# mehrnazmo/VIforSSMs

Measured on AMD Instinct MI355X. Metric: latent-state transitions/sec (batch_dims×T per step), AR(1) T=5000, 1/2/4/8 GPU, higher is better.
Workload: dtype bf16

## Files before the change

viforssms_amd/csrc/flow_v5.hip:

```cpp
#include "flow5_api.hpp"

#ifndef VISSM_FLOW5_NS
#define VISSM_FLOW5_NS flow5
#define VISSM_FLOW5_BASE_UNIT 1
#endif

#include <cstdlib>
#ifndef VISSM_ABL_STORES
#define VISSM_ABL_STORES 0
#endif

namespace vissm {
namespace VISSM_FLOW5_NS {

constexpr int P = 16;
constexpr int HP = 64;
constexpr int S = 16;
constexpr int NW = 4;
constexpr int NT = 64 * NW;
constexpr int UW = 128;
constexpr int DTH = 56;

typedef __bf16 bf4 __attribute__((ext_vector_type(4)));
typedef __bf16 bf8 __attribute__((ext_vector_type(8)));
// ... 1057 lines not shown
  }
}

constexpr int NW2 = 8;
constexpr int NT2 = 64 * NW2;
__device__ __forceinline__ float swap_hi_lo(float v) {
  const auto r = __builtin_amdgcn_permlane32_swap(__builtin_bit_cast(unsigned, v), __builtin_bit_cast(unsigned, v),
                                                  false, false);
  return __builtin_bit_cast(float, static_cast<unsigned>(r[1]));
}
constexpr int KP2 = 8;
#ifndef VISSM_NODU_FENCES
#define VISSM_NODU_FENCES 1
#endif
template <bool FZ>
__device__ __forceinline__ void fence2() {
  if constexpr (FZ) fence();
}
#ifndef VISSM_BWD2_AHEAD
#define VISSM_BWD2_AHEAD 2
#endif
#ifndef VISSM_BWD2_AHEAD_VAR
#define VISSM_BWD2_AHEAD_VAR 6
#endif
#ifndef VISSM_BWD2_TAIL_DU
#define VISSM_BWD2_TAIL_DU 5
#endif
#ifndef VISSM_BWD2_TAIL_FZ
#define VISSM_BWD2_TAIL_FZ 59
#endif
#ifndef VISSM_BWD2_TAIL_NODU
#define VISSM_BWD2_TAIL_NODU 4
#endif
constexpr int kSgMfma = 0x008, kSgDsRead = 0x100;
template <int ID, int N, int M>
__device__ __forceinline__ void sg_batch() {
  __builtin_amdgcn_sched_group_barrier(kSgDsRead, N, ID);
#pragma unroll
  for (int i = 0; i < N; ++i) __builtin_amdgcn_sched_group_barrier(kSgMfma, M, ID);
}
template <int ID, int NR, int NM>
__device__ __forceinline__ void sg_seq() {
  __builtin_amdgcn_sched_group_barrier(kSgDsRead, NR, ID);
  __builtin_amdgcn_sched_group_barrier(kSgMfma, NM, ID);
}

__device__ __forceinline__ bf8 cat8(bf4 a, bf4 b) {
  return __builtin_shufflevector(a, b, 0, 1, 2, 3, 4, 5, 6, 7);
}
__device__ __forceinline__ bf8 tr_frag2(const __bf16* img, int hb, int g, int c) {
  return cat8(tr_read(img, hb, g, c), tr_read(img + P * HP, hb, g, c));
}

template <bool FZ, bool DU, bool TF, int NPR = 1, bool SB = false>
__global__ __launch_bounds__(NT2, 2) void bwd2_kernel(KArgs a, const float* __restrict__ u, const float* __restrict__ C,
                                                      const float* __restrict__ tht, const float* __restrict__ gout,
                                                      const float* __restrict__ dls, const bf8* __restrict__ img,
                                                      const float* __restrict__ cst, float* __restrict__ du,
                                                      float* __restrict__ dC_slab, float* __restrict__ dth_slab,
                                                      float* __restrict__ dW_slab, float* __restrict__ halo,
                                                      const u4* __restrict__ thf, FzArgs fz = FzArgs{}) {
  static_assert(!SB || NPR == 2, "the split backward chain goes with the split recompute");
  constexpr int NH = 1, KB = 1, JB = 1, NP = 1;
  constexpr bool LOF = NPR == 2 && !kLoFoldOff;
  constexpr bool AH =
      VISSM_BWD2_AHEAD && NPR == 1 && (FZ || TF) && (VISSM_BWD2_AHEAD_VAR & (FZ ? 4 : DU ? 2 : 1)) != 0;
  constexpr int TAIL = (VISSM_BWD2_AHEAD >= 2 && NPR == 1 && TF)
                           ? (FZ ? VISSM_BWD2_TAIL_FZ : DU ? VISSM_BWD2_TAIL_DU : VISSM_BWD2_TAIL_NODU) : 0;
  constexpr int PO = FZ ? P - 1 : P;
  constexpr int QW2 = P + KP2;
  constexpr int UWN = NPR == 2 ? 48 : 64;
  __shared__ Shared<NH, KB, JB, NP> sh;
  __shared__ __bf16 timg[NW2][2][2 * P * HP];
  __shared__ float dthl[NW2][S][DTH];
  __shared__ __attribute__((aligned(16))) float dths[NW2][4];
  __shared__ float carry[NW2][S][KP2];
  __shared__ float uwin[NW2][2][UWN];
  __shared__ float gwin[NW2][2][P];
  __shared__ float gsc[NPR == 2 ? 1 : NW2][2][P];
  __shared__ float dscr[NW2][2][KP2][QW2];
  constexpr bool ZLS = FZ && NPR == 1;
  __shared__ float zls[ZLS ? NW2 : 1][ZLS ? S : 1][P];
  constexpr int RO = NPR == 2 ? 10 : 0, NLO = RO + (SB ? 10 : 0);
  __shared__ bf8 slo[NLO > 0 ? NLO : 1][64];
  __shared__ bf8 swe[NPR == 2 ? 4 : 1][16];
  __shared__ float zcar[FZ ? NW2 : 1][FZ ? S : 1];
  if constexpr (NPR == 2) {
    constexpr int NFR = Shared<NH, KB, JB, NP>::NFR;
    for (int i = threadIdx.x; i < NFR * 64; i += NT2) sh.img[i >> 6][0][i & 63] = img[((i >> 6) * 2) * 64 + (i & 63)];
    for (int i = threadIdx.x; i < NLO * 64; i += NT2) {
      const int j = i >> 6;
      const int f = j < 8 ? j
                  : j < 10 ? 16 * NH + 4 * KB + 2 * JB + (j - 8)
                  : j < 18 ? 8 * NH + (j - 10)
                           : 16 * NH + 4 * KB + (j - 18);
      slo[j][i & 63] = img[(f * 2 + 1) * 64 + (i & 63)];
    }
    for (int i = threadIdx.x; i < 4 * 16; i += NT2) swe[i >> 4][i & 15] = img[((16 * NH + (i >> 4)) * 2 + 1) * 64 + (i & 15)];
    for (int i = threadIdx.x; i < Shared<NH, KB, JB, NP>::NCST; i += NT2) sh.cst[i] = cst[i];
  } else {
    load_shared<NH, KB, JB, NP, NT2>(sh, img, cst);
  }
  if constexpr (FZ) {
    if constexpr (ZLS)
      for (int i = threadIdx.x; i < NW2 * S * P; i += NT2) (&zls[0][0][0])[i] = 0.f;
    for (int i = threadIdx.x; i < NW2 * S; i += NT2) (&zcar[0][0])[i] = 0.f;
  }
  for (int i = threadIdx.x; i < NW2 * S * DTH; i += NT2) (&dthl[0][0][0])[i] = 0.f;
  for (int i = threadIdx.x; i < NW2 * S * KP2; i += NT2) (&carry[0][0][0])[i] = 0.f;
  for (int i = threadIdx.x; i < NW2 * 2 * KP2 * QW2; i += NT2) (&dscr[0][0][0][0])[i] = 0.f;
  __syncthreads();
// ... 3 lines not shown
  const int chn = __builtin_amdgcn_readfirstlane(item % a.n_chunks);
  if (grp >= a.n_groups) return;
  const int m_lo = chn * a.CH, m_hi = min(a.Lh, m_lo + a.CH);
  const int b_lo = grp * a.S, nb = min(a.S, a.B - b_lo);
  __bf16* const im0 = timg[w][0];
  __bf16* const im1 = timg[w][1];
  const unsigned* whp = reinterpret_cast<const unsigned*>(&sh.cst[NH * HP]);

  f4 dW[4][4], dWe[4], dWh[4];
#pragma unroll
  for (int i = 0; i < 4; ++i) {
#pragma unroll
    for (int o = 0; o < 4; ++o) dW[i][o] = f4{0.f, 0.f, 0.f, 0.f};
    dWe[i] = f4{0.f, 0.f, 0.f, 0.f};
    dWh[i] = f4{0.f, 0.f, 0.f, 0.f};
  }
  const int fwc = 16 * NH + 4 * KB;
  bf8 sel_p;
#pragma unroll
  for (int jj = 0; jj < 8; ++jj) sel_p[jj] = (__bf16)((4 * g + (jj & 3) == c) ? 1.f : 0.f);

  const float ldl = (!FZ && lane < nb) ? dls[b_lo + lane] : 0.f;
  float lt0 = 0.f, lt1 = 0.f, lis = 0.f;
  if constexpr (FZ) {
    if (lane < nb) {
      const float* tp = fz.theta + static_cast<size_t>(b_lo + lane) * 3;
      lt0 = tp[0];
      lt1 = tp[1];
      lis = __expf(-tp[2]);
    }
  }
  const int m_start = (FZ && chn > 0) ? m_lo - PO : m_lo;
  const int nu = a.k + P;
  for (int m0 = m_start; m0 < m_hi; m0 += PO) {
    const bool discard = FZ && m0 < m_lo;
    const int nP = discard ? 0 : min(PO, m_hi - m0), t0 = m0;
    const int nZ = FZ ? min(P, a.Lh - m0) : nP;
    f4 dCa[4];
#pragma unroll
    for (int rb = 0; rb < 4; ++rb) dCa[rb] = f4{0.f, 0.f, 0.f, 0.f};
    float fz_yt = 0.f, fz_bt = 0.f;
    if constexpr (FZ) {
      const int wo = min(max(m0 + c - 1, 0), fz.M - 1);
      fz_yt = fz.obs[wo];
      fz_bt = fz.bin[wo];
    }
    for (int bl = 0; bl < nb; bl += 2) {
      fence2<FZ || (!DU && VISSM_NODU_FENCES)>();
      const bool two = bl + 1 < nb;
      const int blv[2] = {bl, two ? bl + 1 : bl};
      const int bv[2] = {b_lo + blv[0], b_lo + blv[1]};
      f4 X[2][4];
      bf8 tfr[2];
      float fz_yp = fz_yt, fz_bp = fz_bt, fz_zc[2] = {0.f, 0.f};
      {
        float uv[2], gv[2] = {0.f, 0.f};
#pragma unroll
        for (int cb = 0; cb < 2; ++cb) {
          const float* ub = u + static_cast<size_t>(bv[cb]) * a.pL;
          uv[cb] = lane < nu ? ub[clampi(t0 + lane, a.L)] : 0.f;
          if constexpr (!FZ) {
            if (lane < P) gv[cb] = gout[static_cast<size_t>(bv[cb]) * a.pLo + clampi(t0 + lane, a.Lout)];
          }
        }
        if (!two) gv[1] = 0.f;
        const f4* crow = reinterpret_cast<const f4*>(C + static_cast<size_t>(m0 + clampi(c, nZ)) * HP) + g;
        f4 cr[4], tr[2][4];
        if constexpr (TF) {
#pragma unroll
          for (int cb = 0; cb < 2; ++cb) tfr[cb] = __builtin_bit_cast(bf8, thf[2 * static_cast<size_t>(bv[cb]) + (g & 1)]);
        }
#pragma unroll
        for (int rb = 0; rb < 4; ++rb) {
          cr[rb] = crow[4 * rb];
          if constexpr (!TF) {
#pragma unroll
            for (int cb = 0; cb < 2; ++cb)
              tr[cb][rb] = (reinterpret_cast<const f4*>(tht + static_cast<size_t>(bv[cb]) * HP) + g)[4 * rb];
          }
        }
        __builtin_amdgcn_sched_barrier(0);
#pragma unroll
        for (int cb = 0; cb < 2; ++cb) {
          if (UWN == 64 || lane < UWN) uwin[w][cb][lane] = uv[cb];
          if (lane < P) gwin[w][cb][lane] = gv[cb];
#pragma unroll
          for (int rb = 0; rb < 4; ++rb) X[cb][rb] = TF ? cr[rb] : cr[rb] + tr[cb][rb];
        }
        if constexpr (FZ) {
          fz_zc[0] = zcar[w][blv[0]];
          fz_zc[1] = zcar[w][blv[1]];
        }
      }
      u2 i0p[2][4];
      u2 d0p[2][4], d1p[2][4];
      float mu[2], rr[2];
      float uk_e = 0.f;
      {
        f4 acc[2][4];
        fence2<FZ || (!DU && VISSM_NODU_FENCES)>();
        const int gu = (LOF && g == 1) ? 0 : g;
        Fr8<NP> uf[2] = {u_frag<NP>(uwin[w][0], 1, 0, gu, c), u_frag<NP>(uwin[w][1], 1, 0, gu, c)};
        if constexpr (TF) {
          if (g >= 2) {
            uf[0].h = tfr[0];
            uf[1].h = tfr[1];
          }
        }
        if constexpr (AH) {
          bf8 we[4];
#pragma unroll
          for (int ob = 0; ob < 4; ++ob) we[ob] = sh.img[16 * NH + ob][0][lane];
          if constexpr ((TAIL & 8) != 0) __builtin_amdgcn_sched_barrier(0);
#pragma unroll
          for (int ob = 0; ob < 4; ++ob)
#pragma unroll
            for (int cb = 0; cb < 2; ++cb) acc[cb][ob] = mfma32(we[ob], uf[cb].h, X[cb][ob]);
          if constexpr ((TAIL & 8) == 0) sg_batch<1, 4, 2>();
        } else {
#pragma unroll
          for (int ob = 0; ob < 4; ++ob) {
            const Fr8<NP> wf = wfrag(sh, 16 * NH + ob, lane);
            bf8 wel = {};
            if constexpr (NPR == 2 && !LOF) {
              const bf8 v = swe[ob][c];
              if (g == 0) wel = v;
            }
#pragma unroll
            for (int cb = 0; cb < 2; ++cb) {
              acc[cb][ob] = X[cb][ob];
              if constexpr (NPR == 2 && !LOF) acc[cb][ob] = mfma32(wel, uf[cb].h, acc[cb][ob]);
              acc[cb][ob] = mm<NP>(wf, uf[cb], acc[cb][ob]);
            }
          }
        }
#pragma unroll
        for (int cb = 0; cb < 2; ++cb)
#pragma unroll
          for (int rb = 0; rb < 4; ++rb) {
            float e[4] = {0.f, 0.f, 0.f, 0.f};
#pragma unroll
            for (int r = 0; r < 4; ++r) {
              if (VISSM_DERIV16 >= 1) X[cb][rb][r] = 4 * rb + r < NR ? elu_dv(acc[cb][rb][r], e[r]) : 0.f;
              else X[cb][rb][r] = 4 * rb + r < NR ? elu_fast<true>(acc[cb][rb][r]) : 0.f;
            }
            if (VISSM_DERIV16 >= 1) {
              d0p[cb][rb] = u2{pk_f16(e[0], e[1]), 4 * rb + 2 < NR ? pk_f16(e[2], e[3]) : 0u};
              pin_pair(d0p[cb][rb]);
            }
          }
        fence2<FZ || (!DU && VISSM_NODU_FENCES)>();
#pragma unroll
        for (int cb = 0; cb < 2; ++cb) {
          if (g == 3) X[cb][3][3] = 1.f;
#pragma unroll
          for (int ob = 0; ob < 4; ++ob) acc[cb][ob] = f4{0.f, 0.f, 0.f, 0.f};
        }
#pragma unroll
        for (int ks = 0; ks < 2; ++ks) {
          Fr8<NP> xf[2] = {chain_frag<NP>(X[0], ks), chain_frag<NP>(X[1], ks)};
          if constexpr (AH) {
            bf8 wq[4];
#pragma unroll
            for (int ob = 0; ob < 4; ++ob) wq[ob] = sh.img[ob * 2 + ks][0][lane];
#pragma unroll
            for (int ob = 0; ob < 4; ++ob)
#pragma unroll
              for (int cb = 0; cb < 2; ++cb) acc[cb][ob] = mfma32(wq[ob], xf[cb].h, acc[cb][ob]);
            if (ks == 0) sg_batch<2, 4, 2>();
            else sg_batch<3, 4, 2>();
          } else {
#pragma unroll
            for (int ob = 0; ob < 4; ++ob) {
              const Fr8<NP> wf = wfrag(sh, ob * 2 + ks, lane);
#pragma unroll
              for (int cb = 0; cb < 2; ++cb) {
                if constexpr (NPR == 2) acc[cb][ob] = mfma32(slo[ob * 2 + ks][lane], xf[cb].h, acc[cb][ob]);
                acc[cb][ob] = mm<NP>(wf, xf[cb], acc[cb][ob]);
              }
            }
          }
        }
#pragma unroll
        for (int cb = 0; cb < 2; ++cb) {
          put_image<NP>(im0 + cb * P * HP, nullptr, X[cb], g, c);
          if (VISSM_DERIV16 == 0) {
#pragma unroll
            for (int rb = 0; rb < 4; ++rb) i0p[cb][rb] = u2{cvt2(X[cb][rb][0], X[cb][rb][1]), cvt2(X[cb][rb][2], X[cb][rb][3])};
          }
        }
#pragma unroll
        for (int cb = 0; cb < 2; ++cb)
#pragma unroll
          for (int rb = 0; rb < 4; ++rb) {
            float e[4] = {0.f, 0.f, 0.f, 0.f};
#pragma unroll
            for (int r = 0; r < 4; ++r) {
              if (VISSM_DERIV16 >= 2) X[cb][rb][r] = 4 * rb + r < NR ? elu_dv(acc[cb][rb][r], e[r]) : 0.f;
              else X[cb][rb][r] = 4 * rb + r < NR ? elu_fast<true>(acc[cb][rb][r]) : 0.f;
            }
            if (VISSM_DERIV16 >= 2) {
              d1p[cb][rb] = u2{pk_f16(e[0], e[1]), 4 * rb + 2 < NR ? pk_f16(e[2], e[3]) : 0u};
              pin_pair(d1p[cb][rb]);
            }
          }
        fence2<FZ || (!DU && VISSM_NODU_FENCES)>();
        const int fh = 16 * NH + 4 * KB + 2 * JB;
        f4 d[2] = {f4{0.f, 0.f, 0.f, 0.f}, f4{0.f, 0.f, 0.f, 0.f}};
#pragma unroll
        for (int cb = 0; cb < 2; ++cb)
          if (g == 3) X[cb][3][3] = 1.f;
        if constexpr (FZ && (TAIL & 32) != 0) uk_e = uwin[w][g >> 1][c + a.k];
        if constexpr (AH) {
          const bf8 wh[2] = {sh.img[fh][0][lane], sh.img[fh + 1][0][lane]};
#pragma unroll
          for (int ks = 0; ks < 2; ++ks)
#pragma unroll
            for (int cb = 0; cb < 2; ++cb) d[cb] = mfma32(wh[ks], chain_frag<NP>(X[cb], ks).h, d[cb]);
          sg_batch<4, 2, 2>();
        } else {
#pragma unroll
          for (int ks = 0; ks < 2; ++ks) {
            const Fr8<NP> wf = wfrag(sh, fh + ks, lane);
#pragma unroll
            for (int cb = 0; cb < 2; ++cb) {
              const Fr8<NP> xk = chain_frag<NP>(X[cb], ks);
              if constexpr (NPR == 2 && !LOF) d[cb] = mfma32(slo[8 + ks][lane], xk.h, d[cb]);
              d[cb] = mm<NP>(wf, xk, d[cb]);
            }
          }
        }
#pragma unroll
        for (int cb = 0; cb < 2; ++cb) {
          mu[cb] = LOF ? d[cb][0] + d[cb][2] : d[cb][0];
          rr[cb] = LOF ? d[cb][1] + d[cb][3] : d[cb][1];
          put_image<NP>(im1 + cb * P * HP, nullptr, X[cb], g, c);
        }
      }
      const bool pv = c < nP;
      float gmu[2], gr[2];
      float lsv[2] = {0.f, 0.f};
      if constexpr (FZ) {
        const int hs = g >> 1;
        const bool hv = hs == 0 || two;
        const float mu_h = hs ? mu[1] : mu[0], rr_h = hs ? rr[1] : rr[0];
        const float sig_h = softplus_fast(rr_h) + 1e-10f;
        const float uk = (TAIL & 32) ? uk_e : uwin[w][hs][c + a.k];
        const float x = uk * sig_h + mu_h;
        float xp = row_prev(x);
        const float xn = row_next(x);
        if (c == 0) xp = hs ? fz_zc[1] : fz_zc[0];
        const int bl2 = hs ? blv[1] : blv[0];
        const float th0 = hs ? lane_f(lt0, blv[1]) : lane_f(lt0, blv[0]);
        const float th1 = hs ? lane_f(lt1, blv[1]) : lane_f(lt1, blv[0]);
        const float is = hs ? lane_f(lis, blv[1]) : lane_f(lis, blv[0]);
        const int t = m0 + c;
        const float fh = (pv && t < fz.M) ? 1.f : 0.f;
        const float ft = (pv && t >= 1) ? 1.f : 0.f;
        const float bp = fz_bp * ft;
        const float zt = fh * (xn - th1 * x - th0) * is;
        const float zp = ft * (x - th1 * xp - th0) * is;
        const float de = th1 * zt * is - zp * is - bp * (x - fz_yp) * (fz.iosd * fz.iosd);
        const float gmu_h = hv ? -fz.scale * de : 0.f;
        const float lsg = (t0 + c >= a.Lout - a.n_logsig) ? __builtin_amdgcn_logf(sig_h) * kLn2 : 0.f;
        if ((g & 1) == 0) {
          if constexpr (NPR == 1) gwin[w][hs][c] = gmu_h;
          if (pv && hv) {
            if constexpr (!(VISSM_ABL_STORES & 1)) fz.x[static_cast<size_t>(b_lo + bl2) * (fz.M + 1) + t] = x;
            if constexpr (ZLS) zls[w][bl2][c] += lsg;
          }
        }
        if ((lane & 31) == PO - 1 && (nP == PO || discard) && hv) zcar[w][bl2] = x;
        float dsig = gmu_h * uk;
        if (pv && hv && t0 + c >= a.Lout - a.n_logsig) dsig += -fz.scale * rcp_f(sig_h);
        const float gr_h = dsig * sigmoid_fast(rr_h);
        if ((g & 1) == 0) {
          if constexpr (NPR == 2) {
            if constexpr (DU) gwin[w][hs][c] = gmu_h * sig_h;
          } else {
            gsc[w][hs][c] = sig_h;
          }
        }
        gmu[0] = gmu_h;
        gr[0] = gr_h;
        gmu[1] = swap_hi_lo(gmu_h);
        gr[1] = swap_hi_lo(gr_h);
        if constexpr (!ZLS) {
          const float lsv_h = (pv && hv) ? lsg : 0.f;
          lsv[0] = lsv_h;
          lsv[1] = swap_hi_lo(lsv_h);
        }
#pragma unroll
        for (int cb = 0; cb < 2; ++cb) {
          if (g == 1) {
            const int off = timg_off(c, 4 * 3 + 1);
            *reinterpret_cast<u2*>(im1 + cb * P * HP + off) = u2{cvt2(X[cb][3][0], gmu[cb]), cvt2(gr[cb], X[cb][3][3])};
          }
        }
      } else {
        float sig[2];
#pragma unroll
        for (int cb = 0; cb < 2; ++cb) {
          sig[cb] = softplus_fast(rr[cb]) + 1e-10f;
          gmu[cb] = pv ? gwin[w][cb][c] : 0.f;
        }
#pragma unroll
        for (int cb = 0; cb < 2; ++cb) {
          const float dl = lane_f(ldl, blv[cb]);
          float dsig = gmu[cb] * uwin[w][cb][c + a.k];
          if (pv && (cb == 0 || two) && t0 + c >= a.Lout - a.n_logsig) dsig += dl * rcp_f(sig[cb]);
          gr[cb] = dsig * sigmoid_fast(rr[cb]);
          if (g == 0) {
            if constexpr (NPR == 2) {
              if constexpr (DU) gwin[w][cb][c] = gmu[cb] * sig[cb];
            } else {
              gsc[w][cb][c] = sig[cb];
            }
          }
          if (g == 1) {
            const int off = timg_off(c, 4 * 3 + 1);
            *reinterpret_cast<u2*>(im1 + cb * P * HP + off) = u2{cvt2(X[cb][3][0], gmu[cb]), cvt2(gr[cb], X[cb][3][3])};
          }
        }
      }
      fence2<FZ || (!DU && VISSM_NODU_FENCES)>();
      bf8 i1f[4];
#pragma unroll
      for (int hb = 0; hb < 4; ++hb) i1f[hb] = tr_frag2(im1, hb, g, c);
      if constexpr (!AH) {
#pragma unroll
        for (int hb = 0; hb < 4; ++hb) dWh[hb] = mfma32(i1f[hb], i1f[3], dWh[hb]);
      }
      f4 D[2][4];
      {
        unsigned wvh[4], wvl[4];
#pragma unroll
        for (int rb = 0; rb < 4; ++rb) {
          wvh[rb] = whp[16 * rb + c];
          if constexpr (SB) wvl[rb] = whp[HP + 16 * rb + c];
        }
        const bool g0 = g == 0;
#pragma unroll
        for (int cb = 0; cb < 2; ++cb) {
          const bf4 gf2 = __builtin_bit_cast(bf4, u2{cvt2(g0 ? gmu[cb] : 0.f, g0 ? gr[cb] : 0.f), 0u});
#pragma unroll
          for (int rb = 0; rb < 4; ++rb) {
            const bf4 wa = __builtin_bit_cast(bf4, u2{g0 ? wvh[rb] : 0u, 0u});
            f4 d0 = f4{0.f, 0.f, 0.f, 0.f};
            if constexpr (SB) d0 = mfma16(__builtin_bit_cast(bf4, u2{g0 ? wvl[rb] : 0u, 0u}), gf2, d0);
            D[cb][rb] = mfma16(wa, gf2, d0);
          }
        }
        fence2<FZ || (!DU && VISSM_NODU_FENCES)>();
#pragma unroll
        for (int cb = 0; cb < 2; ++cb) {
#pragma unroll
          for (int rb = 0; rb < 4; ++rb)
#pragma unroll
// ... 37 lines not shown
#pragma unroll
            for (int cb = 0; cb < 2; ++cb) {
              if constexpr (SB) dX[cb][ib] = mfma32(slo[RO + ib * 2 + ks][lane], df[cb].h, dX[cb][ib]);
              dX[cb][ib] = mm<NP>(wb, df[cb], dX[cb][ib]);
            }
          }
        }
      }
      fence2<FZ || (!DU && VISSM_NODU_FENCES)>();
      {
        bf8 dzf[4];
#pragma unroll
        for (int ob = 0; ob < 4; ++ob) dzf[ob] = tr_frag2(im1, ob, g, c);
        if constexpr (AH) {
          bf8 xa[4];
#pragma unroll
          for (int ib = 0; ib < 4; ++ib) xa[ib] = tr_frag2(im0, ib, g, c);
#pragma unroll
          for (int ib = 0; ib < 4; ++ib)
#pragma unroll
            for (int ob = 0; ob < 4; ++ob) dW[ib][ob] = mfma32(xa[ib], dzf[ob], dW[ib][ob]);
          sg_seq<9, 16, 16>();
        } else {
#pragma unroll
          for (int ib = 0; ib < 4; ++ib) {
            const bf8 xa = tr_frag2(im0, ib, g, c);
#pragma unroll
            for (int ob = 0; ob < 4; ++ob) dW[ib][ob] = mfma32(xa, dzf[ob], dW[ib][ob]);
          }
        }
      }
      bf8 uaf_e = {};
      if constexpr ((TAIL & 4) != 0) {
        const Fr4<NP> ua = ua_frag<NP>(uwin[w][0], 1, 0, g, c), ub = ua_frag<NP>(uwin[w][1], 1, 0, g, c);
        uaf_e = cat8(ua.h, ub.h);
      }
#pragma unroll
      for (int cb = 0; cb < 2; ++cb)
#pragma unroll
        for (int rb = 0; rb < 4; ++rb) {
          if (VISSM_DERIV16 >= 1) {
#pragma unroll
            for (int r = 0; r < 4; ++r) D[cb][rb][r] = 4 * rb + r < NR ? mul_h(dX[cb][rb][r], d0p[cb][rb][r >> 1], r & 1) : 0.f;
          } else {
            const f4 x = {__builtin_bit_cast(float, i0p[cb][rb][0] << 16), __builtin_bit_cast(float, i0p[cb][rb][0] & 0xffff0000u),
                          __builtin_bit_cast(float, i0p[cb][rb][1] << 16), __builtin_bit_cast(float, i0p[cb][rb][1] & 0xffff0000u)};
#pragma unroll
            for (int r = 0; r < 4; ++r) D[cb][rb][r] = 4 * rb + r < NR ? dX[cb][rb][r] * elu_d(x[r]) : 0.f;
          }
        }
      f4 dcn[2] = {f4{0.f, 0.f, 0.f, 0.f}, f4{0.f, 0.f, 0.f, 0.f}};
      if constexpr (DU && AH) {
        const bf8 wc[2] = {sh.img[fwc][0][lane], sh.img[fwc + 1][0][lane]};
#pragma unroll
        for (int ks = 0; ks < 2; ++ks)
#pragma unroll
          for (int cb = 0; cb < 2; ++cb) dcn[cb] = mfma32(wc[ks], chain_frag<NP>(D[cb], ks).h, dcn[cb]);
        sg_batch<7, 2, 2>();
      } else if constexpr (DU) {
#pragma unroll
        for (int ks = 0; ks < 2; ++ks) {
          const Fr8<NP> wc = wfrag(sh, fwc + ks, lane);
#pragma unroll
          for (int cb = 0; cb < 2; ++cb) {
            const Fr8<NP> dk = chain_frag<NP>(D[cb], ks);
            if constexpr (SB) dcn[cb] = mfma32(slo[RO + 8 + ks][lane], dk.h, dcn[cb]);
            dcn[cb] = mm<NP>(wc, dk, dcn[cb]);
          }
        }
      }
      if constexpr (FZ && !ZLS) {
#pragma unroll
        for (int cb = 0; cb < 2; ++cb) {
          const float hi = bf16_hi(lsv[cb]);
          D[cb][3][1] = g == 0 ? hi : (g == 1 ? lsv[cb] - hi : 0.f);
        }
      }
#pragma unroll
      for (int cb = 0; cb < 2; ++cb) put_image<NP>(im1 + cb * P * HP, nullptr, D[cb], g, c);
      if constexpr (DU) {
        if (g < KP2 / 4) {
#pragma unroll
          for (int cb = 0; cb < 2; ++cb)
#pragma unroll
            for (int r = 0; r < 4; ++r) dscr[w][cb][4 * g + r][c + 4 * g + r] = dcn[cb][r];
        }
      }
      float dut[KP2], dug = 0.f, dus = 0.f, duc = 0.f;
      const auto du_rows = [&]() {
        const int cbq = lane >> 5, q = lane & 31;
        const int qc = q < QW2 ? q : QW2 - 1;
#pragma unroll
        for (int j = 0; j < KP2; ++j) dut[j] = dscr[w][cbq][j][qc];
      };
      const auto du_terms = [&]() {
        const int cbq = lane >> 5, q = lane & 31;
        const int oqc = min(max(q - a.k, 0), P - 1);
        dug = gwin[w][cbq][oqc];
        dus = gsc[w][cbq][oqc];
        duc = carry[w][cbq ? blv[1] : blv[0]][q & (KP2 - 1)];
      };
      if constexpr (DU && (TAIL & 1) != 0) du_rows();
      if constexpr (DU && (TAIL & 2) != 0) du_terms();
      fence2<FZ || (!DU && VISSM_NODU_FENCES)>();
      {
        const unsigned one2 = 0x3F803F80u;
        bf8 uaf = uaf_e;
        if constexpr ((TAIL & 4) == 0) {
          const Fr4<NP> ua = ua_frag<NP>(uwin[w][0], 1, 0, g, c), ub = ua_frag<NP>(uwin[w][1], 1, 0, g, c);
          uaf = cat8(ua.h, ub.h);
        }
        bf8 bcomb = uaf;
        {
          const unsigned ta_ = c - 8 == (blv[0] & 7) ? one2 : 0u, tb_ = (two && c - 8 == (blv[1] & 7)) ? one2 : 0u;
          if (c >= 8) bcomb = __builtin_bit_cast(bf8, u4{ta_, ta_, tb_, tb_});
        }
        if constexpr (AH) {
          bf8 ta[4];
#pragma unroll
          for (int hb = 0; hb < 4; ++hb) ta[hb] = tr_frag2(im1, hb, g, c);
#pragma unroll
          for (int hb = 0; hb < 4; ++hb) {
            dWe[hb] = mfma32(ta[hb], bcomb, dWe[hb]);
            dCa[hb] = mfma32(ta[hb], sel_p, dCa[hb]);
          }
          sg_seq<10, 8, 8>();
        } else {
#pragma unroll
          for (int hb = 0; hb < 4; ++hb) {
            const bf8 ta = tr_frag2(im1, hb, g, c);
            dWe[hb] = mfma32(ta, bcomb, dWe[hb]);
            dCa[hb] = mfma32(ta, sel_p, dCa[hb]);
          }
        }
      }
      {
        if ((bl & 7) == 6 || bl + 2 >= nb) {
          const int smp = (bl & ~7) + c - 8;
          if (c >= 8 && smp < nb) {
            float* base = &dthl[w][smp][4 * g];
            f4* dp[4];
#pragma unroll
// ... 3 lines not shown
#pragma unroll
            for (int hb = 0; hb < 4; ++hb) o[hb] = *dp[hb];
#pragma unroll
            for (int hb = 0; hb < 4; ++hb) *dp[hb] = o[hb] + dWe[hb];
          }
#pragma unroll
          for (int hb = 0; hb < 4; ++hb)
            if (c >= 8) dWe[hb] = f4{0.f, 0.f, 0.f, 0.f};
        }
      }
      if constexpr (DU) {
        fence2<FZ || (!DU && VISSM_NODU_FENCES)>();
        const int cbq = lane >> 5, q = lane & 31;
        const int lim = nP + a.k;
        const bool act = q < lim && (cbq == 0 || two);
        const int blq = cbq ? blv[1] : blv[0];
        float v = 0.f;
        if (act) {
          const int qc = q < QW2 ? q : QW2 - 1;
          float t[KP2];
#pragma unroll
          for (int j = 0; j < KP2; ++j) t[j] = (TAIL & 1) ? dut[j] : dscr[w][cbq][j][qc];
#pragma unroll
          for (int w2 = 1; w2 < KP2; w2 *= 2)
#pragma unroll
            for (int j = 0; j + w2 < KP2; j += 2 * w2) t[j] += t[j + w2];
          v = t[0];
          const int oq2 = q - a.k;
          if constexpr ((TAIL & 2) != 0) {
            if (oq2 >= 0 && oq2 < nP) v += dug * dus;
            if (q < a.k) v += duc;
          } else {
            if (oq2 >= 0 && oq2 < nP)
              v += NPR == 2 ? gwin[w][cbq][oq2] : gwin[w][cbq][oq2] * gsc[w][cbq][oq2];
            if (q < a.k) v += carry[w][blq][q];
          }
        }
        if (act) {
          float* const dur = du + static_cast<size_t>(b_lo + blq) * a.pL + t0;
          if (q < nP) {
            if constexpr (!(VISSM_ABL_STORES & 2)) dur[q] = v;
          } else {
            carry[w][blq][q - nP] = v;
          }
        }
      }
    }
    if (c < nP && !(VISSM_ABL_STORES & 4)) {
      const size_t row = (static_cast<size_t>(grp) * a.Lh + m0 + c) * a.H;
      if (a.dc16) {
        __bf16* dcs = reinterpret_cast<__bf16*>(dC_slab) + row;
#pragma unroll
        for (int rb = 0; rb < 4; ++rb)
#pragma unroll
          for (int r = 0; r < 4; ++r) {
            const int h = swz(16 * rb + 4 * g + r);
            if (h < a.H) dcs[h] = static_cast<__bf16>(dCa[rb][r] * kLog2e);
          }
      } else {
        float* dcs = dC_slab + row;
#pragma unroll
        for (int rb = 0; rb < 4; ++rb)
#pragma unroll
          for (int r = 0; r < 4; ++r) {
            const int h = swz(16 * rb + 4 * g + r);
            if (h < a.H) dcs[h] = dCa[rb][r] * kLog2e;
          }
      }
    }
  }

  if constexpr (FZ) {
    if (lane < nb) {
      float v = 0.f;
      if constexpr (!ZLS) {
        v = dthl[w][lane][49] + dthl[w][lane][53];
      } else {
#pragma unroll
        for (int cc = 0; cc < P; ++cc) v += zls[w][lane][cc];
// ... 32 lines not shown
      for (int r = 0; r < 4; ++r) {
        const int hi = swz(16 * ib + 4 * g + r), ho = swz(16 * ob + c);
        if (ho < H) {
          if (hi < H) ws[off_w + hi * H + ho] = dW[ib][ob][r];
          else if (hi == 63) ws[off_b + ho] = dW[ib][ob][r] * kLog2e;
        }
      }
  for (int i = lane; i < 2 * NH * H; i += 64) ws[off_b + NH * H + i] = 0.f;
  const int off_h = off_b + 3 * NH * H;
  const int oh = c - 5;
  if (oh == 0 || oh == 1) {
#pragma unroll
    for (int hb = 0; hb < 4; ++hb)
#pragma unroll
      for (int r = 0; r < 4; ++r) {
        const int h = swz(16 * hb + 4 * g + r);
        if (h < H) ws[off_h + h * 2 + oh] = dWh[hb][r] * kLn2;
        else if (h == 63) ws[off_h + 2 * H + oh] = dWh[hb][r];
      }
  }
}

template <bool TF, int NP, int NH, int JB, int NWF = NW, bool LOF = false>
__global__ __launch_bounds__(64 * NWF, 2) void fwd2_kernel(KArgs a, const float* __restrict__ u,
                                                                  const float* __restrict__ C,
                                                                  const float* __restrict__ tht,
                                                                  const bf8* __restrict__ img,
                                                                  const float* __restrict__ cst,
                                                                  float* __restrict__ u_next,
                                                                  float* __restrict__ ls_slab,
                                                                  const u4* __restrict__ thf) {
  constexpr int KB = (JB + 1) / 2;
  __shared__ Shared<NH, KB, JB, NP> sh;
  __shared__ float uwin[NWF][2][64 * KB];
  load_shared<NH, KB, JB, NP, 64 * NWF>(sh, img, cst);
  {
    const int r = __builtin_amdgcn_readfirstlane(blockIdx.x / a.ncu) & 3;
    if (r == 1) __builtin_amdgcn_s_setprio(1);
    else if (r == 2) __builtin_amdgcn_s_setprio(2);
    else if (r == 3) __builtin_amdgcn_s_setprio(3);
  }
  __syncthreads();
  const int w = threadIdx.x >> 6, lane = threadIdx.x & 63, c = lane & 15, g = lane >> 4;
  const int item = __builtin_amdgcn_readfirstlane(blockIdx.x * NWF + w);
  if (item >= a.n_items) return;
  const int grp = item / a.n_chunks, ch = item % a.n_chunks;
  const int m_lo = ch * a.CH, m_hi = min(a.Lh, m_lo + a.CH);
  const int b_lo = grp * a.S, nb = min(a.S, a.B - b_lo);
  constexpr bool HIREG = NWF == NW;
  constexpr int NWR = HIREG ? 8 * NH + 4 * KB + 2 : 1;
  bf8 wr[NWR];
  constexpr bool HIDREG = !HIREG && LOF && VISSM_X2_HIDREG;
  bf8 wrh[HIDREG ? 8 * NH : 1];
  if constexpr (HIDREG) {
#pragma unroll
    for (int i = 0; i < 8 * NH; ++i) wrh[i] = sh.img[i][0][lane];
  }
  if constexpr (HIREG) {
#pragma unroll
    for (int i = 0; i < 8 * NH; ++i) wr[i] = sh.img[i][0][lane];
#pragma unroll
    for (int i = 0; i < 4 * KB; ++i) wr[8 * NH + i] = sh.img[16 * NH + i][0][lane];
#pragma unroll
    for (int i = 0; i < 2; ++i) wr[8 * NH + 4 * KB + i] = sh.img[16 * NH + 4 * KB + 2 * JB + i][0][lane];
  }
  auto W = [&](int f, int i) -> Fr8<NP> {
    Fr8<NP> r;
    if constexpr (HIREG) r.h = wr[i];
    else if (HIDREG && f < 8 * NH) r.h = wrh[HIDREG ? f : 0];
    else r.h = sh.img[f][0][lane];
    if constexpr (NP == 2) r.l = sh.img[f][1][lane];
    return r;
  };
  auto mmw = [](const Fr8<NP>& a, const bf8& b, f4 cc) -> f4 {
    if constexpr (NP == 2) cc = mfma32(a.l, b, cc);
    return mfma32(a.h, b, cc);
  };
  const int ss = NH == 1 ? 1 : a.s;
  const bool swp = NH == 1 ? false : a.swap_out != 0;
  const int nu = ss * P + a.k;
  for (int bl = 0; bl < nb; bl += 2) {
    const bool two = bl + 1 < nb;
    const int bv[2] = {b_lo + bl, b_lo + (two ? bl + 1 : bl)};
    float ls[2] = {0.f, 0.f};
    bf8 tfr[2];
    if constexpr (TF) {
#pragma unroll
      for (int cb = 0; cb < 2; ++cb) tfr[cb] = __builtin_bit_cast(bf8, thf[2 * static_cast<size_t>(bv[cb]) + (g & 1)]);
    }
    for (int m0 = m_lo; m0 < m_hi; m0 += P) {
      const int nP = min(P, m_hi - m0), t0 = ss * m0;
      f4 X[2][4];
      {
        float uv[2][KB];
#pragma unroll
        for (int cb = 0; cb < 2; ++cb)
#pragma unroll
          for (int i = 0; i < KB; ++i)
            uv[cb][i] = 64 * i + lane < nu ? u[static_cast<size_t>(bv[cb]) * a.pL + clampi(t0 + 64 * i + lane, a.L)] : 0.f;
        const f4* crow = reinterpret_cast<const f4*>(C + static_cast<size_t>(m0 + clampi(c, nP)) * HP) + g;
        f4 cr[4], tr[2][4];
#pragma unroll
        for (int rb = 0; rb < 4; ++rb) {
          cr[rb] = crow[4 * rb];
          if constexpr (!TF) {
#pragma unroll
            for (int cb = 0; cb < 2; ++cb)
              tr[cb][rb] = (reinterpret_cast<const f4*>(tht + static_cast<size_t>(bv[cb]) * HP) + g)[4 * rb];
          }
        }
        __builtin_amdgcn_sched_barrier(0);
#pragma unroll
        for (int cb = 0; cb < 2; ++cb) {
#pragma unroll
          for (int i = 0; i < KB; ++i) uwin[w][cb][64 * i + lane] = uv[cb][i];
#pragma unroll
          for (int rb = 0; rb < 4; ++rb) X[cb][rb] = TF ? cr[rb] : cr[rb] + tr[cb][rb];
        }
      }
      f4 acc[2][4];
      {
#pragma unroll
        for (int kb = 0; kb < KB; ++kb) {
          const int gu = (LOF && g == 1) ? 0 : g;
          bf8 uf[2] = {u_frag<1>(uwin[w][0], ss, kb, gu, c).h, u_frag<1>(uwin[w][1], ss, kb, gu, c).h};
          if constexpr (TF) {
            if (g >= 2) {
              uf[0] = tfr[0];
              uf[1] = tfr[1];
            }
          }
#pragma unroll
          for (int ob = 0; ob < 4; ++ob) {
            if constexpr (LOF) {
              const bf8 wh = HIREG ? wr[8 * NH + 4 * kb + ob] : sh.img[16 * NH + 4 * kb + ob][0][lane];
#pragma unroll
              for (int cb = 0; cb < 2; ++cb) acc[cb][ob] = mfma32(wh, uf[cb], kb == 0 ? X[cb][ob] : acc[cb][ob]);
            } else {
              const Fr8<NP> wf = W(16 * NH + 4 * kb + ob, 8 * NH + 4 * kb + ob);
#pragma unroll
              for (int cb = 0; cb < 2; ++cb) acc[cb][ob] = mmw(wf, uf[cb], kb == 0 ? X[cb][ob] : acc[cb][ob]);
            }
          }
        }
      }
#pragma unroll
      for (int cb = 0; cb < 2; ++cb)
#pragma unroll
        for (int rb = 0; rb < 4; ++rb)
#pragma unroll
          for (int r = 0; r < 4; ++r) X[cb][rb][r] = 4 * rb + r < NR ? elu_fast<true>(acc[cb][rb][r]) : 0.f;
#pragma unroll
      for (int l = 0; l < NH; ++l) {
#pragma unroll
        for (int cb = 0; cb < 2; ++cb) {
          if (g == 3) X[cb][3][3] = 1.f;
#pragma unroll
          for (int ob = 0; ob < 4; ++ob) acc[cb][ob] = f4{0.f, 0.f, 0.f, 0.f};
        }
#pragma unroll
        for (int ks = 0; ks < 2; ++ks) {
          const bf8 xf[2] = {chain_frag<1>(X[0], ks).h, chain_frag<1>(X[1], ks).h};
#pragma unroll
          for (int ob = 0; ob < 4; ++ob) {
            const Fr8<NP> wf = W(l * 8 + ob * 2 + ks, l * 8 + ob * 2 + ks);
#pragma unroll
            for (int cb = 0; cb < 2; ++cb) acc[cb][ob] = mmw(wf, xf[cb], acc[cb][ob]);
          }
        }
#pragma unroll
        for (int cb = 0; cb < 2; ++cb)
#pragma unroll
          for (int rb = 0; rb < 4; ++rb)
#pragma unroll
            for (int r = 0; r < 4; ++r) X[cb][rb][r] = 4 * rb + r < NR ? elu_fast<true>(acc[cb][rb][r]) : 0.f;
      }
#pragma unroll
      for (int cb = 0; cb < 2; ++cb)
        if (g == 3) X[cb][3][3] = 1.f;
      const int fh = 16 * NH + 4 * KB + 2 * JB;
      f4 d[2] = {f4{0.f, 0.f, 0.f, 0.f}, f4{0.f, 0.f, 0.f, 0.f}};
#pragma unroll
      for (int ks = 0; ks < 2; ++ks) {
        if constexpr (LOF) {
          const bf8 wh = HIREG ? wr[8 * NH + 4 * KB + ks] : sh.img[fh + ks][0][lane];
#pragma unroll
          for (int cb = 0; cb < 2; ++cb) d[cb] = mfma32(wh, chain_frag<1>(X[cb], ks).h, d[cb]);
        } else {
          const Fr8<NP> wf = W(fh + ks, 8 * NH + 4 * KB + ks);
#pragma unroll
          for (int cb = 0; cb < 2; ++cb) d[cb] = mmw(wf, chain_frag<1>(X[cb], ks).h, d[cb]);
        }
      }
      if constexpr (LOF) {
#pragma unroll
        for (int cb = 0; cb < 2; ++cb) {
          d[cb][0] += d[cb][2];
          d[cb][1] += d[cb][3];
        }
      }
      if (g == 0 && c < nP) {
#pragma unroll
        for (int cb = 0; cb < 2; ++cb) {
          if (cb == 1 && !two) break;
          const float sg = softplus_fast(d[cb][1]) + 1e-10f;
          const int oq = ss * c + (ss - 1), o = t0 + oq;
          float* ob = u_next + static_cast<size_t>(bv[cb]) * a.pLo;
          ob[swp ? (o ^ 1) : o] = uwin[w][cb][oq + a.k] * sg + d[cb][0];
          if (ss == 2) {
            const int oe = t0 + 2 * c;
            ob[swp ? (oe ^ 1) : oe] = uwin[w][cb][2 * c + a.k];
          }
          if (o >= a.Lout - a.n_logsig) ls[cb] += __builtin_amdgcn_logf(sg) * kLn2;
        }
      }
    }
#pragma unroll
    for (int cb = 0; cb < 2; ++cb) {
      const float v = wave_sum(ls[cb]);
      if (lane == 0 && (cb == 0 || two)) ls_slab[static_cast<size_t>(ch) * a.B + bv[cb]] = v;
    }
  }
}

constexpr int NW3 = 4;
constexpr int NT3 = 64 * NW3;

__device__ __forceinline__ void put_pairs(__bf16* img, const u2 (&v)[4], int g, int c) {
#pragma unroll
  for (int rb = 0; rb < 4; ++rb) *reinterpret_cast<u2*>(img + timg_off(c, 4 * rb + g)) = v[rb];
}
__device__ __forceinline__ f4 unpack_pair(u2 v) {
  return f4{__builtin_bit_cast(float, v[0] << 16), __builtin_bit_cast(float, v[0] & 0xffff0000u),
            __builtin_bit_cast(float, v[1] << 16), __builtin_bit_cast(float, v[1] & 0xffff0000u)};
}

template <int JB, bool S2, bool DU>
__global__ __launch_bounds__(NT3, 1) void bwd2n_kernel(KArgs a, const float* __restrict__ u, const float* __restrict__ C,
                                                       const float* __restrict__ tht, const float* __restrict__ gout,
                                                       const float* __restrict__ dls, const bf8* __restrict__ img,
                                                       const float* __restrict__ cst, float* __restrict__ du,
                                                       float* __restrict__ dC_slab, float* __restrict__ dth_slab,
                                                       float* __restrict__ dW_slab, float* __restrict__ halo) {
  constexpr int NH = 3, KB = (JB + 1) / 2, NP = 1;
  static_assert(JB <= 2 || !S2, "k > 32: stride 1 only");
  constexpr int s = S2 ? 2 : 1;
  constexpr int KP = 16 * JB;
  constexpr bool DIAG = JB > 2;
  constexpr bool AACC = VISSM_BWD2N_AACC && JB <= 2;
  constexpr bool DV = VISSM_DERIV16 >= 2 && JB <= 2 && !DU;
  constexpr int KR = JB == 1 ? 16 : JB == 2 ? 24 : KP;
  constexpr int QWR = DIAG ? P + 1 : s * P + KR;
  constexpr int UWN = KB == 1 ? 64 : 128;
  __shared__ Shared<NH, KB, JB, NP> sh;
  __shared__ __bf16 timg[NW3][2][2 * P * HP];
  __shared__ float dthl[NW3][S][DTH];
// ... 931 lines not shown
```

Measured before the change: 4.425 billion.

## Prefetch u/gout windows into double-buffered LDS via global_load_lds DMA

Replaces the per-iteration global loads of the u and gout windows, which went through registers and then into shared memory, with asynchronous global_load_lds_dword transfers. These write straight into a double-buffered LDS window, issued one iteration ahead in the backward and forward flow kernels. Each iteration waits on vmcnt(0) before using the current buffer, then issues the next tile's loads at a chosen site so they overlap with compute. This hides global memory latency at the cost of doubled LDS for the windows, inline asm that manipulates m0 and exec, and a blanket vmcnt wait that may also stall on unrelated loads.

```diff
diff --git a/viforssms_amd/csrc/flow_v5.hip b/viforssms_amd/csrc/flow_v5.hip
--- a/viforssms_amd/csrc/flow_v5.hip
+++ b/viforssms_amd/csrc/flow_v5.hip
@@ -1113,6 +1113,56 @@
 #ifndef VISSM_BWD2_TAIL_NODU
 #define VISSM_BWD2_TAIL_NODU 4
 #endif
+#ifndef VISSM_STAGE_AHEAD
+#define VISSM_STAGE_AHEAD 1
+#endif
+#ifndef VISSM_STAGE_AHEAD_VAR
+#define VISSM_STAGE_AHEAD_VAR 12
+#endif
+#ifndef VISSM_STAGE_SITE_DU
+#define VISSM_STAGE_SITE_DU 0
+#endif
+#ifndef VISSM_STAGE_SITE_FZ
+#define VISSM_STAGE_SITE_FZ 2
+#endif
+__device__ __forceinline__ unsigned lds_addr(const void* p) {
+  return __builtin_amdgcn_readfirstlane(
+      static_cast<unsigned>(reinterpret_cast<size_t>((__attribute__((address_space(3))) const void*)p)));
+}
+__device__ __forceinline__ void lds_dma_pair(unsigned long long mask0, unsigned long long mask1, unsigned voff,
+                                             const float* base0, const float* base1, unsigned dst0, unsigned dst1) {
+  unsigned keep_m0;
+  unsigned long long keep_exec;
+  asm volatile(
+      "s_nop 4\n\t"
+      "s_mov_b32 %0, m0\n\t"
+      "s_and_saveexec_b64 %1, %2\n\t"
+      "s_mov_b32 m0, %7\n\t"
+      "s_nop 0\n\t"
+      "global_load_lds_dword %4, %5\n\t"
+      "s_and_b64 exec, %1, %3\n\t"
+      "s_mov_b32 m0, %8\n\t"
+      "s_nop 0\n\t"
+      "global_load_lds_dword %4, %6\n\t"
+      "s_mov_b64 exec, %1\n\t"
+      "s_mov_b32 m0, %0"
+      : "=&s"(keep_m0), "=&s"(keep_exec)
+      : "s"(mask0), "s"(mask1), "v"(voff), "s"(base0), "s"(base1), "s"(dst0), "s"(dst1)
+      : "memory", "scc");
+}
+__device__ __forceinline__ unsigned long long lanes_below(int n, bool on) {
+  return on ? (n >= 64 ? ~0ull : (1ull << n) - 1ull) : 0ull;
+}
+template <int N>
+__device__ __forceinline__ void stage_windows(const float* src, int pitch, int len, int b0, int b1, int t0, int n,
+                                              int lane, float (*win)[N], bool on, bool both) {
+  const unsigned long long m = lanes_below(n, on);
+  lds_dma_pair(m, both ? m : 0ull, 4u * static_cast<unsigned>(clampi(t0 + lane, len)),
+               src + static_cast<size_t>(b0) * pitch, src + static_cast<size_t>(b1) * pitch, lds_addr(win[0]),
+               lds_addr(win[1]));
+}
+__device__ __forceinline__ void stage_wait() { asm volatile("s_waitcnt vmcnt(0)" ::: "memory"); }
+
 constexpr int kSgMfma = 0x008, kSgDsRead = 0x100;
 template <int ID, int N, int M>
 __device__ __forceinline__ void sg_batch() {
@@ -1133,6 +1183,8 @@
   return cat8(tr_read(img, hb, g, c), tr_read(img + P * HP, hb, g, c));
 }
 
+#define VISSM_UW (*(STG ? &uwin[pw + w] : &uwin[w]))
+#define VISSM_GW (*(STGG ? &gwin[pw + w] : &gwin[w]))
 template <bool FZ, bool DU, bool TF, int NPR = 1, bool SB = false>
 __global__ __launch_bounds__(NT2, 2) void bwd2_kernel(KArgs a, const float* __restrict__ u, const float* __restrict__ C,
                                                       const float* __restrict__ tht, const float* __restrict__ gout,
@@ -1156,8 +1208,12 @@
   __shared__ float dthl[NW2][S][DTH];
   __shared__ __attribute__((aligned(16))) float dths[NW2][4];
   __shared__ float carry[NW2][S][KP2];
-  __shared__ float uwin[NW2][2][UWN];
-  __shared__ float gwin[NW2][2][P];
+  constexpr bool STG = VISSM_STAGE_AHEAD && NPR == 1 && TF && UWN == 64 &&
+                       (VISSM_STAGE_AHEAD_VAR & (FZ ? 8 : DU ? 4 : 2)) != 0;
+  constexpr bool STGG = STG && !FZ;
+  constexpr int SITE = FZ ? VISSM_STAGE_SITE_FZ : VISSM_STAGE_SITE_DU;
+  __shared__ float uwin[STG ? 2 * NW2 : NW2][2][UWN];
+  __shared__ float gwin[STGG ? 2 * NW2 : NW2][2][P];
   __shared__ float gsc[NPR == 2 ? 1 : NW2][2][P];
   __shared__ float dscr[NW2][2][KP2][QW2];
   constexpr bool ZLS = FZ && NPR == 1;
@@ -1227,6 +1283,20 @@
   }
   const int m_start = (FZ && chn > 0) ? m_lo - PO : m_lo;
   const int nu = a.k + P;
+  int par = 0;
+  if constexpr (STG) {
+    if (lane >= nu) {
+#pragma unroll
+      for (int cb = 0; cb < 2; ++cb) {
+        uwin[w][cb][lane] = 0.f;
+        uwin[NW2 + w][cb][lane] = 0.f;
+      }
+    }
+    stage_windows(u, a.pL, a.L, b_lo, b_lo + (1 < nb ? 1 : 0), m_start, nu, lane, uwin[w], m_start < m_hi, true);
+    if constexpr (!FZ)
+      stage_windows(gout, a.pLo, a.Lout, b_lo, b_lo + (1 < nb ? 1 : 0), m_start, P, lane, gwin[w], m_start < m_hi,
+                    1 < nb);
+  }
   for (int m0 = m_start; m0 < m_hi; m0 += PO) {
     const bool discard = FZ && m0 < m_lo;
     const int nP = discard ? 0 : min(PO, m_hi - m0), t0 = m0;
@@ -1245,20 +1315,39 @@
       const bool two = bl + 1 < nb;
       const int blv[2] = {bl, two ? bl + 1 : bl};
       const int bv[2] = {b_lo + blv[0], b_lo + blv[1]};
+      int pw = 0;
+      if constexpr (STG) {
+        stage_wait();
+        pw = par * NW2;
+        asm volatile("" : "+s"(pw));
+      }
+      const auto stage_next = [&]() {
+        const bool lastp = bl + 2 >= nb, more = !lastp || m0 + PO < m_hi;
+        const int ms = (lastp && more) ? m0 + PO : m0, bs = lastp ? (more ? 0 : bl) : bl + 2;
+        const int b0 = b_lo + bs, b1 = b_lo + (bs + 1 < nb ? bs + 1 : bs);
+        __builtin_amdgcn_sched_barrier(0);
+        stage_windows(u, a.pL, a.L, b0, b1, ms, nu, lane, uwin[NW2 - pw + w], more, true);
+        if constexpr (STGG)
+          stage_windows(gout, a.pLo, a.Lout, b0, b1, ms, P, lane, gwin[NW2 - pw + w], more, bs + 1 < nb);
+        __builtin_amdgcn_sched_barrier(0);
+      };
+      (void)stage_next;
       f4 X[2][4];
       bf8 tfr[2];
       float fz_yp = fz_yt, fz_bp = fz_bt, fz_zc[2] = {0.f, 0.f};
       {
-        float uv[2], gv[2] = {0.f, 0.f};
-#pragma unroll
-        for (int cb = 0; cb < 2; ++cb) {
-          const float* ub = u + static_cast<size_t>(bv[cb]) * a.pL;
-          uv[cb] = lane < nu ? ub[clampi(t0 + lane, a.L)] : 0.f;
-          if constexpr (!FZ) {
-            if (lane < P) gv[cb] = gout[static_cast<size_t>(bv[cb]) * a.pLo + clampi(t0 + lane, a.Lout)];
-          }
-        }
-        if (!two) gv[1] = 0.f;
+        float uv[2] = {0.f, 0.f}, gv[2] = {0.f, 0.f};
+        if constexpr (!STG) {
+#pragma unroll
+          for (int cb = 0; cb < 2; ++cb) {
+            const float* ub = u + static_cast<size_t>(bv[cb]) * a.pL;
+            uv[cb] = lane < nu ? ub[clampi(t0 + lane, a.L)] : 0.f;
+            if constexpr (!FZ) {
+              if (lane < P) gv[cb] = gout[static_cast<size_t>(bv[cb]) * a.pLo + clampi(t0 + lane, a.Lout)];
+            }
+          }
+          if (!two) gv[1] = 0.f;
+        }
         const f4* crow = reinterpret_cast<const f4*>(C + static_cast<size_t>(m0 + clampi(c, nZ)) * HP) + g;
         f4 cr[4], tr[2][4];
         if constexpr (TF) {
@@ -1275,10 +1364,19 @@
           }
         }
         __builtin_amdgcn_sched_barrier(0);
+        if constexpr (STG) {
+          if constexpr (!FZ) {
+            if (!two && lane < P) VISSM_GW[1][lane] = 0.f;
+          } else {
+            asm volatile("" : "+v"(fz_yp), "+v"(fz_bp));
+          }
+        }
 #pragma unroll
         for (int cb = 0; cb < 2; ++cb) {
-          if (UWN == 64 || lane < UWN) uwin[w][cb][lane] = uv[cb];
-          if (lane < P) gwin[w][cb][lane] = gv[cb];
+          if constexpr (!STG) {
+            if (UWN == 64 || lane < UWN) VISSM_UW[cb][lane] = uv[cb];
+            if (lane < P) VISSM_GW[cb][lane] = gv[cb];
+          }
 #pragma unroll
           for (int rb = 0; rb < 4; ++rb) X[cb][rb] = TF ? cr[rb] : cr[rb] + tr[cb][rb];
         }
@@ -1295,7 +1393,7 @@
         f4 acc[2][4];
         fence2<FZ || (!DU && VISSM_NODU_FENCES)>();
         const int gu = (LOF && g == 1) ? 0 : g;
-        Fr8<NP> uf[2] = {u_frag<NP>(uwin[w][0], 1, 0, gu, c), u_frag<NP>(uwin[w][1], 1, 0, gu, c)};
+        Fr8<NP> uf[2] = {u_frag<NP>(VISSM_UW[0], 1, 0, gu, c), u_frag<NP>(VISSM_UW[1], 1, 0, gu, c)};
         if constexpr (TF) {
           if (g >= 2) {
             uf[0].h = tfr[0];
@@ -1345,6 +1443,7 @@
             }
           }
         fence2<FZ || (!DU && VISSM_NODU_FENCES)>();
+        if constexpr (STG && SITE == 0) stage_next();
 #pragma unroll
         for (int cb = 0; cb < 2; ++cb) {
           if (g == 3) X[cb][3][3] = 1.f;
@@ -1405,7 +1504,7 @@
 #pragma unroll
         for (int cb = 0; cb < 2; ++cb)
           if (g == 3) X[cb][3][3] = 1.f;
-        if constexpr (FZ && (TAIL & 32) != 0) uk_e = uwin[w][g >> 1][c + a.k];
+        if constexpr (FZ && (TAIL & 32) != 0) uk_e = VISSM_UW[g >> 1][c + a.k];
         if constexpr (AH) {
           const bf8 wh[2] = {sh.img[fh][0][lane], sh.img[fh + 1][0][lane]};
 #pragma unroll
@@ -1440,7 +1539,7 @@
         const bool hv = hs == 0 || two;
         const float mu_h = hs ? mu[1] : mu[0], rr_h = hs ? rr[1] : rr[0];
         const float sig_h = softplus_fast(rr_h) + 1e-10f;
-        const float uk = (TAIL & 32) ? uk_e : uwin[w][hs][c + a.k];
+        const float uk = (TAIL & 32) ? uk_e : VISSM_UW[hs][c + a.k];
         const float x = uk * sig_h + mu_h;
         float xp = row_prev(x);
         const float xn = row_next(x);
@@ -1459,7 +1558,7 @@
         const float gmu_h = hv ? -fz.scale * de : 0.f;
         const float lsg = (t0 + c >= a.Lout - a.n_logsig) ? __builtin_amdgcn_logf(sig_h) * kLn2 : 0.f;
         if ((g & 1) == 0) {
-          if constexpr (NPR == 1) gwin[w][hs][c] = gmu_h;
+          if constexpr (NPR == 1) VISSM_GW[hs][c] = gmu_h;
           if (pv && hv) {
             if constexpr (!(VISSM_ABL_STORES & 1)) fz.x[static_cast<size_t>(b_lo + bl2) * (fz.M + 1) + t] = x;
             if constexpr (ZLS) zls[w][bl2][c] += lsg;
@@ -1471,7 +1570,7 @@
         const float gr_h = dsig * sigmoid_fast(rr_h);
         if ((g & 1) == 0) {
           if constexpr (NPR == 2) {
-            if constexpr (DU) gwin[w][hs][c] = gmu_h * sig_h;
+            if constexpr (DU) VISSM_GW[hs][c] = gmu_h * sig_h;
           } else {
             gsc[w][hs][c] = sig_h;
           }
@@ -1497,17 +1596,17 @@
 #pragma unroll
         for (int cb = 0; cb < 2; ++cb) {
           sig[cb] = softplus_fast(rr[cb]) + 1e-10f;
-          gmu[cb] = pv ? gwin[w][cb][c] : 0.f;
+          gmu[cb] = pv ? VISSM_GW[cb][c] : 0.f;
         }
 #pragma unroll
         for (int cb = 0; cb < 2; ++cb) {
           const float dl = lane_f(ldl, blv[cb]);
-          float dsig = gmu[cb] * uwin[w][cb][c + a.k];
+          float dsig = gmu[cb] * VISSM_UW[cb][c + a.k];
           if (pv && (cb == 0 || two) && t0 + c >= a.Lout - a.n_logsig) dsig += dl * rcp_f(sig[cb]);
           gr[cb] = dsig * sigmoid_fast(rr[cb]);
           if (g == 0) {
             if constexpr (NPR == 2) {
-              if constexpr (DU) gwin[w][cb][c] = gmu[cb] * sig[cb];
+              if constexpr (DU) VISSM_GW[cb][c] = gmu[cb] * sig[cb];
             } else {
               gsc[w][cb][c] = sig[cb];
             }
@@ -1519,6 +1618,7 @@
         }
       }
       fence2<FZ || (!DU && VISSM_NODU_FENCES)>();
+      if constexpr (STG && SITE == 2) stage_next();
       bf8 i1f[4];
 #pragma unroll
       for (int hb = 0; hb < 4; ++hb) i1f[hb] = tr_frag2(im1, hb, g, c);
@@ -1622,7 +1722,7 @@
       }
       bf8 uaf_e = {};
       if constexpr ((TAIL & 4) != 0) {
-        const Fr4<NP> ua = ua_frag<NP>(uwin[w][0], 1, 0, g, c), ub = ua_frag<NP>(uwin[w][1], 1, 0, g, c);
+        const Fr4<NP> ua = ua_frag<NP>(VISSM_UW[0], 1, 0, g, c), ub = ua_frag<NP>(VISSM_UW[1], 1, 0, g, c);
         uaf_e = cat8(ua.h, ub.h);
       }
 #pragma unroll
@@ -1686,7 +1786,7 @@
       const auto du_terms = [&]() {
         const int cbq = lane >> 5, q = lane & 31;
         const int oqc = min(max(q - a.k, 0), P - 1);
-        dug = gwin[w][cbq][oqc];
+        dug = VISSM_GW[cbq][oqc];
         dus = gsc[w][cbq][oqc];
         duc = carry[w][cbq ? blv[1] : blv[0]][q & (KP2 - 1)];
       };
@@ -1697,7 +1797,7 @@
         const unsigned one2 = 0x3F803F80u;
         bf8 uaf = uaf_e;
         if constexpr ((TAIL & 4) == 0) {
-          const Fr4<NP> ua = ua_frag<NP>(uwin[w][0], 1, 0, g, c), ub = ua_frag<NP>(uwin[w][1], 1, 0, g, c);
+          const Fr4<NP> ua = ua_frag<NP>(VISSM_UW[0], 1, 0, g, c), ub = ua_frag<NP>(VISSM_UW[1], 1, 0, g, c);
           uaf = cat8(ua.h, ub.h);
         }
         bf8 bcomb = uaf;
@@ -1767,7 +1867,7 @@
             if (q < a.k) v += duc;
           } else {
             if (oq2 >= 0 && oq2 < nP)
-              v += NPR == 2 ? gwin[w][cbq][oq2] : gwin[w][cbq][oq2] * gsc[w][cbq][oq2];
+              v += NPR == 2 ? VISSM_GW[cbq][oq2] : VISSM_GW[cbq][oq2] * gsc[w][cbq][oq2];
             if (q < a.k) v += carry[w][blq][q];
           }
         }
@@ -1780,6 +1880,7 @@
           }
         }
       }
+      if constexpr (STG) par ^= 1;
     }
     if (c < nP && !(VISSM_ABL_STORES & 4)) {
       const size_t row = (static_cast<size_t>(grp) * a.Lh + m0 + c) * a.H;
@@ -1878,7 +1979,9 @@
                                                                   const u4* __restrict__ thf) {
   constexpr int KB = (JB + 1) / 2;
   __shared__ Shared<NH, KB, JB, NP> sh;
-  __shared__ float uwin[NWF][2][64 * KB];
+  constexpr bool STG = VISSM_STAGE_AHEAD && (VISSM_STAGE_AHEAD_VAR & 1) != 0 && TF && NP == 1 && NH == 1 && JB == 1 &&
+                       NWF == NW && !LOF;
+  __shared__ float uwin[STG ? 2 * NWF : NWF][2][64 * KB];
   load_shared<NH, KB, JB, NP, 64 * NWF>(sh, img, cst);
   {
     const int r = __builtin_amdgcn_readfirstlane(blockIdx.x / a.ncu) & 3;
@@ -1925,6 +2028,17 @@
   const int ss = NH == 1 ? 1 : a.s;
   const bool swp = NH == 1 ? false : a.swap_out != 0;
   const int nu = ss * P + a.k;
+  int par = 0;
+  if constexpr (STG) {
+    if (lane >= nu) {
+#pragma unroll
+      for (int cb = 0; cb < 2; ++cb) {
+        uwin[w][cb][lane] = 0.f;
+        uwin[NWF + w][cb][lane] = 0.f;
+      }
+    }
+    stage_windows(u, a.pL, a.L, b_lo, b_lo + (1 < nb ? 1 : 0), m_lo, nu, lane, uwin[w], nb > 0 && m_lo < m_hi, true);
+  }
   for (int bl = 0; bl < nb; bl += 2) {
     const bool two = bl + 1 < nb;
     const int bv[2] = {b_lo + bl, b_lo + (two ? bl + 1 : bl)};
@@ -1937,13 +2051,21 @@
     for (int m0 = m_lo; m0 < m_hi; m0 += P) {
       const int nP = min(P, m_hi - m0), t0 = ss * m0;
       f4 X[2][4];
+      int pw = 0;
+      if constexpr (STG) {
+        stage_wait();
+        pw = par * NWF;
+        asm volatile("" : "+s"(pw));
+      }
       {
         float uv[2][KB];
-#pragma unroll
-        for (int cb = 0; cb < 2; ++cb)
-#pragma unroll
-          for (int i = 0; i < KB; ++i)
-            uv[cb][i] = 64 * i + lane < nu ? u[static_cast<size_t>(bv[cb]) * a.pL + clampi(t0 + 64 * i + lane, a.L)] : 0.f;
+        if constexpr (!STG) {
+#pragma unroll
+          for (int cb = 0; cb < 2; ++cb)
+#pragma unroll
+            for (int i = 0; i < KB; ++i)
+              uv[cb][i] = 64 * i + lane < nu ? u[static_cast<size_t>(bv[cb]) * a.pL + clampi(t0 + 64 * i + lane, a.L)] : 0.f;
+        }
         const f4* crow = reinterpret_cast<const f4*>(C + static_cast<size_t>(m0 + clampi(c, nP)) * HP) + g;
         f4 cr[4], tr[2][4];
 #pragma unroll
@@ -1958,8 +2080,10 @@
         __builtin_amdgcn_sched_barrier(0);
 #pragma unroll
         for (int cb = 0; cb < 2; ++cb) {
-#pragma unroll
-          for (int i = 0; i < KB; ++i) uwin[w][cb][64 * i + lane] = uv[cb][i];
+          if constexpr (!STG) {
+#pragma unroll
+            for (int i = 0; i < KB; ++i) VISSM_UW[cb][64 * i + lane] = uv[cb][i];
+          }
 #pragma unroll
           for (int rb = 0; rb < 4; ++rb) X[cb][rb] = TF ? cr[rb] : cr[rb] + tr[cb][rb];
         }
@@ -1969,7 +2093,7 @@
 #pragma unroll
         for (int kb = 0; kb < KB; ++kb) {
           const int gu = (LOF && g == 1) ? 0 : g;
-          bf8 uf[2] = {u_frag<1>(uwin[w][0], ss, kb, gu, c).h, u_frag<1>(uwin[w][1], ss, kb, gu, c).h};
+          bf8 uf[2] = {u_frag<1>(VISSM_UW[0], ss, kb, gu, c).h, u_frag<1>(VISSM_UW[1], ss, kb, gu, c).h};
           if constexpr (TF) {
             if (g >= 2) {
               uf[0] = tfr[0];
@@ -1990,6 +2114,14 @@
           }
         }
       }
+      if constexpr (STG) {
+        const bool lastt = m0 + P >= m_hi, more = !lastt || bl + 2 < nb;
+        const int bs = (lastt && more) ? bl + 2 : bl, ms = lastt ? (more ? m_lo : m0) : m0 + P;
+        __builtin_amdgcn_sched_barrier(0);
+        stage_windows(u, a.pL, a.L, b_lo + bs, b_lo + (bs + 1 < nb ? bs + 1 : bs), ms, nu, lane,
+                      uwin[NWF - pw + w], more, true);
+        __builtin_amdgcn_sched_barrier(0);
+      }
 #pragma unroll
       for (int cb = 0; cb < 2; ++cb)
 #pragma unroll
@@ -2052,14 +2184,15 @@
           const float sg = softplus_fast(d[cb][1]) + 1e-10f;
           const int oq = ss * c + (ss - 1), o = t0 + oq;
           float* ob = u_next + static_cast<size_t>(bv[cb]) * a.pLo;
-          ob[swp ? (o ^ 1) : o] = uwin[w][cb][oq + a.k] * sg + d[cb][0];
+          ob[swp ? (o ^ 1) : o] = VISSM_UW[cb][oq + a.k] * sg + d[cb][0];
           if (ss == 2) {
             const int oe = t0 + 2 * c;
-            ob[swp ? (oe ^ 1) : oe] = uwin[w][cb][2 * c + a.k];
+            ob[swp ? (oe ^ 1) : oe] = VISSM_UW[cb][2 * c + a.k];
           }
           if (o >= a.Lout - a.n_logsig) ls[cb] += __builtin_amdgcn_logf(sg) * kLn2;
         }
       }
+      if constexpr (STG) par ^= 1;
     }
 #pragma unroll
     for (int cb = 0; cb < 2; ++cb) {
@@ -2068,6 +2201,9 @@
     }
   }
 }
+
+#undef VISSM_UW
+#undef VISSM_GW
 
 constexpr int NW3 = 4;
 constexpr int NT3 = 64 * NW3;
```

Measured after the change: 4.500 billion, median of 6. 1.7% higher.
